# lvxianwei/DeepMerge

Measured on AMD Instinct MI355X. Metric: superpixel-pairs/sec (train step), higher is better.
Workload: dtype bf16; 1 GPU; ShfitScaleFormer_v3 depth [3, 2, 1], scales [32, 64, 128, 256] x 4ch (256x256x4 patches), 32 pairs/GPU/step, fwd+loss+bwd+allreduce+Adam (BASELINE configs[1]); pairs_per_gpu=32, global_batch=32, parallelism=dp1

## Files before the change

### deepmerge_amd/csrc/dm_gemm.hip

```cpp
#include <cstdlib>

#include "dm_common.h"
#include <cstring>

#include "dm_gemm_common.h"
#include "dm_mfma.h"
#include "dm_prof.h"

bool dm_gemm256_plan(GemmParams &p, int layout, int ab_dtype, bool can_split, long long workspace_bytes, int user_split);
void dm_gemm256_launch(const GemmParams &p, int layout, hipStream_t s);
int dm_gemm_ring_plan(GemmParams &p, int layout, int ab_dtype, bool aligned8);
void dm_gemm_ring_launch(const GemmParams &p, int wm, hipStream_t s);
int dm_gemm_w4_plan(GemmParams &p, int layout, int ab_dtype, bool aligned8, bool can_split, long long workspace_bytes);
void dm_gemm_w4_launch(const GemmParams &p, int layout, int grid, hipStream_t s);
int dm_gemm_w4_grouped(GemmParams *ps, int n, hipStream_t s, bool launch, const DmGroupedExtra &x);
long long dm_gemm_w4_grouped_ws_bytes();

namespace {

constexpr int BM = 128, BN = 128;
constexpr int STAGE_BYTES = 16896;
constexpr int NTHREADS = 256;
#ifndef DM_GEMM_LDS_STAGES
#define DM_GEMM_LDS_STAGES 1
#endif
constexpr int LDS_STAGES = DM_GEMM_LDS_STAGES;
constexpr int WG_PER_CU = (LDS_STAGES == 1) ? 3 : 2;


template <typename T, int TM> struct Geo {
  static constexpr int EPC = DmTypeInfo<T>::kPerChunk;
  static constexpr int TILE = 32 * TM;
  static constexpr int BK = 128 / (int)sizeof(T);
  static constexpr int M_ROWB = (sizeof(T) == 2) ? TILE * 2 : (TILE + 4) * 4;
  static constexpr int M_CPR = TILE / EPC;
  static constexpr int M_RPI = NTHREADS / M_CPR;
  static constexpr int K_BYTES = TILE * 128;
  static constexpr int STAGE = (K_BYTES > BK * M_ROWB) ? K_BYTES : BK * M_ROWB;
};

template <int TM> __device__ __forceinline__ int tr_swz(int k) {
  if constexpr (TM == 4) return (k & 3) | (((k >> 3) & 1) << 2);
  else return ((k >> 1) & 1) | (((k >> 3) & 1) << 1);
}

template <int TM> struct OperandView {
  __amdgpu_buffer_rsrc_t rsrc;
  const void *base;
  long long tail_bytes;
  unsigned voff[TM];
  unsigned chunk_k;
};

__device__ __forceinline__ int clamp_records(long long bytes) {
  return (int)(bytes < 0 ? 0 : (bytes > 0x7fffffffLL ? 0x7fffffffLL : bytes));
}

template <typename T, int TM>
__device__ __forceinline__ OperandView<TM> view_kmajor(const T *base, long long ld, int row0, int rows, int K, int t) {
  constexpr int EPC = DmTypeInfo<T>::kPerChunk;
  OperandView<TM> v;
  const int nrows = min(32 * TM, rows - row0);
  const long long bytes = ((long long)(nrows - 1) * ld + K) * (long long)sizeof(T);
  v.rsrc = __builtin_amdgcn_make_buffer_rsrc(const_cast<T *>(base + (long long)row0 * ld), 0, clamp_records(bytes), 0x00020000);
  v.base = nullptr;
  v.tail_bytes = 0;
  v.chunk_k = (t & 7) * EPC;
#pragma unroll
  for (int i = 0; i < TM; ++i) {
    const int row = (t >> 3) + 32 * i;
    const long long off = ((long long)row * ld + v.chunk_k) * (long long)sizeof(T);
    v.voff[i] = (row < nrows) ? (unsigned)off : 0x80000000u;
  }
  return v;
}
template <typename T, int TM>
__device__ __forceinline__ void load_kmajor(u32x4 (&r)[TM], const OperandView<TM> &v, int k0, int kend, long long kphys) {
  const unsigned kill = ((int)(k0 + v.chunk_k) < kend) ? 0u : 0x80000000u;
  const unsigned soff = (unsigned)kphys * (unsigned)sizeof(T);
#pragma unroll
  for (int i = 0; i < TM; ++i) r[i] = __builtin_amdgcn_raw_buffer_load_b128(v.rsrc, v.voff[i] | kill, soff, 0);
}
template <int TM> __device__ __forceinline__ void store_kmajor(char *lds, const u32x4 (&r)[TM], int t) {
  const int c = t & 7;
#pragma unroll
  for (int i = 0; i < TM; ++i) {
    const int row = (t >> 3) + 32 * i;
    *reinterpret_cast<u32x4 *>(lds + row * 128 + ((c ^ (row & 7)) << 4)) = r[i];
  }
}
template <typename T, int TM>
__device__ __forceinline__ OperandView<TM> view_mmajor(const T *base, long long ld, int col0, int cols, int K, int t) {
  using G = Geo<T, TM>;
  OperandView<TM> v;
  v.base = base + col0;
  v.tail_bytes = ((long long)(K - 1) * ld + (cols - col0)) * (long long)sizeof(T);
  v.rsrc = __builtin_amdgcn_make_buffer_rsrc(const_cast<T *>(base), 0, 0, 0x00020000);
  v.chunk_k = 0;
  const int col = (t % G::M_CPR) * G::EPC;
#pragma unroll
  for (int i = 0; i < TM; ++i) {
    const long long k = t / G::M_CPR + G::M_RPI * i;
    v.voff[i] = (col0 + col < cols) ? (unsigned)((k * ld + col) * (long long)sizeof(T)) : 0x80000000u;
  }
  return v;
}
template <typename T, int TM>
__device__ __forceinline__ void load_mmajor(u32x4 (&r)[TM], const OperandView<TM> &v, long long ld, int k0, long long seg_off = 0) {
  const long long skip = (long long)k0 * ld * (long long)sizeof(T);
  const __amdgpu_buffer_rsrc_t rs = __builtin_amdgcn_make_buffer_rsrc(
      const_cast<char *>(reinterpret_cast<const char *>(v.base) + skip + seg_off * (long long)sizeof(T)), 0, clamp_records(v.tail_bytes - skip), 0x00020000);
#pragma unroll
  for (int i = 0; i < TM; ++i) r[i] = __builtin_amdgcn_raw_buffer_load_b128(rs, v.voff[i], 0, 0);
}
template <typename T, int TM> __device__ __forceinline__ void store_mmajor(char *lds, const u32x4 (&r)[TM], int t) {
  using G = Geo<T, TM>;
  const int c = t % G::M_CPR;
#pragma unroll
  for (int i = 0; i < TM; ++i) {
    const int k = t / G::M_CPR + G::M_RPI * i;
    if constexpr (sizeof(T) == 2)
      *reinterpret_cast<u32x4 *>(lds + k * G::M_ROWB + (((c >> 1) ^ tr_swz<TM>(k)) << 5) + ((c & 1) << 4)) = r[i];
    else
      *reinterpret_cast<u32x4 *>(lds + k * G::M_ROWB + (c << 4)) = r[i];
  }
}

__device__ __forceinline__ u32x4 frag_kmajor(const char *lds, int row, int kb, int lane) {
  const int chunk = kb * 4 + (lane >> 4);
  return *reinterpret_cast<const u32x4 *>(lds + row * 128 + ((chunk ^ (row & 7)) << 4));
}
template <typename T, int TM> __device__ __forceinline__ u32x4 frag_mmajor(const char *lds, int col0, int kb, int lane) {
  using G = Geo<T, TM>;
  const int g = lane >> 4;
  u32x4 out;
  if constexpr (sizeof(T) == 2) {
    const int q = (lane >> 2) & 3, p = lane & 3;
    const int col = col0 + 4 * p;
#pragma unroll
    for (int half = 0; half < 2; ++half) {
      const int k = kb * 32 + 8 * g + 4 * half + q;
      const u32x2 w = dm_ds_read_tr16(lds + k * G::M_ROWB + (((col >> 4) ^ tr_swz<TM>(k)) << 5) + ((col & 15) << 1));
      out[2 * half] = w[0];
      out[2 * half + 1] = w[1];
    }
  } else {
    const int i = lane & 15;
#pragma unroll
    for (int j = 0; j < 4; ++j) {
      const int k = kb * 16 + 4 * g + j;
      out[j] = *reinterpret_cast<const unsigned int *>(lds + k * G::M_ROWB + ((col0 + i) << 2));
    }
  }
  return out;
}

template <typename T, int LAYOUT, int TM, bool FOLD = false>
__global__ __launch_bounds__(NTHREADS, (TM == 4 ? WG_PER_CU : 4)) void gemm_kernel(const GemmParams p) {
  using G = Geo<T, TM>;
  constexpr bool A_MMAJOR = (LAYOUT == DM_TN);
  constexpr bool B_MMAJOR = (LAYOUT != DM_NT);
  constexpr int BK = G::BK;
  constexpr int TILE = G::TILE, WT = 16 * TM;
  __shared__ __attribute__((aligned(16))) char smem[2 * LDS_STAGES * G::STAGE];
  auto ldsA = [&](int buf) -> char * { return smem + (2 * (buf % LDS_STAGES)) * G::STAGE; };
// ... 270 lines not shown
    }
    dm_gemm_emit8(p, lo, hi, dm_gemm_row(p, m), n);
  }
}

__global__ void colsum_rows_reduce_kernel(const float *__restrict__ rows, float *__restrict__ out, int M, int R, int accumulate) {
  const int m = blockIdx.x * blockDim.x + threadIdx.x;
  if (m >= M) return;
  float s0 = accumulate ? out[m] : 0.f, s1 = 0.f, s2 = 0.f, s3 = 0.f;
  int r = 0;
  for (; r + 3 < R; r += 4) {
    s0 += rows[(long long)r * M + m];
    s1 += rows[(long long)(r + 1) * M + m];
    s2 += rows[(long long)(r + 2) * M + m];
    s3 += rows[(long long)(r + 3) * M + m];
  }
  for (; r < R; ++r) s0 += rows[(long long)r * M + m];
  out[m] = (s0 + s1) + (s2 + s3);
}

__device__ __forceinline__ void sgemm_small_emit(const GemmParams &p, int m, int n, float v) {
  if (p.bias) v += p.bias[n];
  const long long ro = (long long)m;
  if (p.epilogue == DM_EPI_GELU) {
    if (p.aux) reinterpret_cast<float *>(p.aux)[ro * p.ldaux + n] = v;
    v = dm_gelu(v);
  } else if (p.epilogue == DM_EPI_DGELU) {
    v *= dm_dgelu(reinterpret_cast<const float *>(p.aux)[ro * p.ldaux + n]);
  } else if (p.epilogue == DM_EPI_GELU_GRAD) {
    reinterpret_cast<float *>(p.aux)[ro * p.ldaux + n] = dm_dgelu(v);
    v = dm_gelu(v);
  } else if (p.epilogue == DM_EPI_MUL) {
    v *= reinterpret_cast<const float *>(p.aux)[ro * p.ldaux + n];
  }
  if (p.residual) v += p.residual[ro * p.ldr + n];
  float *c = reinterpret_cast<float *>(p.C) + ro * p.ldc + n;
  if (p.accumulate) v += *c;
  *c = v;
}

template <int LAYOUT, int NW = 4>
__global__ __launch_bounds__(64 * NW) void sgemm_small_kernel(const GemmParams p) {
  __shared__ float sa[NW][32][17], sb[NW][32][17];
  __shared__ float red[NW][16][17];
  const int lane = threadIdx.x & 63, w = threadIdx.x >> 6;
  const int m0 = blockIdx.y * 16, n0 = blockIdx.x * 16;
  const float *A = reinterpret_cast<const float *>(p.A);
  const float *B = reinterpret_cast<const float *>(p.B);
  const int kz0 = gridDim.z > 1 ? blockIdx.z * p.k_per_split : 0, kz1 = gridDim.z > 1 ? min(p.K, kz0 + p.k_per_split) : p.K;
  const int kq = ((kz1 - kz0 + NW - 1) / NW + 31) / 32 * 32;
  const int kbeg = kz0 + w * kq, kend = min(kz1, kbeg + kq);
  const int tx = lane & 15, ty = lane >> 4;
  float acc[4] = {0.f, 0.f, 0.f, 0.f};
  float ra[8], rb[8];
  auto gload = [&](int k0) {
#pragma unroll
    for (int i = 0; i < 8; ++i) {
      const int idx = lane + 64 * i;
      {
        const int r = (LAYOUT == DM_TN) ? (idx & 15) : (idx >> 5), kk = (LAYOUT == DM_TN) ? (idx >> 4) : (idx & 31);
        const int m = m0 + r, k = k0 + kk;
        float v = 0.f;
        if (m < p.M && k < kend) v = (LAYOUT == DM_TN) ? A[(long long)k * p.lda + m] : A[(long long)m * p.lda + k];
        ra[i] = v;
      }
      {
        const int c = (LAYOUT == DM_NT) ? (idx >> 5) : (idx & 15), kk = (LAYOUT == DM_NT) ? (idx & 31) : (idx >> 4);
        const int n = n0 + c, k = k0 + kk;
        float v = 0.f;
        if (n < p.N && k < kend) v = (LAYOUT == DM_NT) ? B[(long long)n * p.ldb + k] : B[(long long)k * p.ldb + n];
        rb[i] = v;
      }
    }
  };
  auto lstore = [&]() {
#pragma unroll
    for (int i = 0; i < 8; ++i) {
      const int idx = lane + 64 * i;
      const int ar = (LAYOUT == DM_TN) ? (idx & 15) : (idx >> 5), ak = (LAYOUT == DM_TN) ? (idx >> 4) : (idx & 31);
      sa[w][ak][ar] = ra[i];
      const int bc = (LAYOUT == DM_NT) ? (idx >> 5) : (idx & 15), bk = (LAYOUT == DM_NT) ? (idx & 31) : (idx >> 4);
      sb[w][bk][bc] = rb[i];
    }
  };
  const int nk = (kq + 31) / 32;
  gload(kbeg);
  for (int it = 0; it < nk; ++it) {
    __syncthreads();
    lstore();
    __syncthreads();
    if (it + 1 < nk) gload(kbeg + (it + 1) * 32);
#pragma unroll
    for (int kk = 0; kk < 32; ++kk) {
      const float bv = sb[w][kk][tx];
#pragma unroll
      for (int j = 0; j < 4; ++j) acc[j] = fmaf(sa[w][kk][4 * ty + j], bv, acc[j]);
    }
  }
#pragma unroll
  for (int j = 0; j < 4; ++j) red[w][4 * ty + j][tx] = acc[j];
  __syncthreads();
  if (threadIdx.x >= 256) return;
  const int om = threadIdx.x >> 4, on = threadIdx.x & 15;
  const int m = m0 + om, n = n0 + on;
  if (m >= p.M || n >= p.N) return;
  float v = (red[0][om][on] + red[1][om][on]) + (red[2][om][on] + red[3][om][on]);
  if constexpr (NW > 4) {
#pragma unroll
    for (int q = 4; q < NW; q += 4) v += (red[q][om][on] + red[q + 1][om][on]) + (red[q + 2][om][on] + red[q + 3][om][on]);
  }
  if (gridDim.z > 1) {
    p.workspace[((long long)blockIdx.z * p.M + m) * p.N + n] = v;
    return;
  }
  sgemm_small_emit(p, m, n, v);
}

__global__ __launch_bounds__(256) void sgemm_small_reduce_kernel(const GemmParams p, int slices) {
  const long long i = (long long)blockIdx.x * 256 + threadIdx.x, mn = (long long)p.M * p.N;
  if (i >= mn) return;
  float v = p.workspace[i];
  int z = 1;
  for (; z + 8 <= slices; z += 8) {
    float t[8];
#pragma unroll
    for (int u = 0; u < 8; ++u) t[u] = p.workspace[(z + u) * mn + i];
#pragma unroll
    for (int u = 0; u < 8; ++u) v += t[u];
  }
  for (; z < slices; ++z) v += p.workspace[z * mn + i];
  sgemm_small_emit(p, (int)(i / p.N), (int)(i % p.N), v);
}

template <typename T, int TM>
void launch_mfma(const GemmParams &p, int layout, int grid, hipStream_t s) {
  if constexpr (sizeof(T) == 2) {
    if (p.k_fold > 0) {
      switch (layout) {
        case DM_NT: hipLaunchKernelGGL((gemm_kernel<T, DM_NT, TM, true>), dim3(grid), dim3(NTHREADS), 0, s, p); break;
        case DM_NN: hipLaunchKernelGGL((gemm_kernel<T, DM_NN, TM, true>), dim3(grid), dim3(NTHREADS), 0, s, p); break;
        default: hipLaunchKernelGGL((gemm_kernel<T, DM_TN, TM, true>), dim3(grid), dim3(NTHREADS), 0, s, p); break;
      }
      return;
    }
  }
  switch (layout) {
    case DM_NT: hipLaunchKernelGGL((gemm_kernel<T, DM_NT, TM>), dim3(grid), dim3(NTHREADS), 0, s, p); break;
    case DM_NN: hipLaunchKernelGGL((gemm_kernel<T, DM_NN, TM>), dim3(grid), dim3(NTHREADS), 0, s, p); break;
    default: hipLaunchKernelGGL((gemm_kernel<T, DM_TN, TM>), dim3(grid), dim3(NTHREADS), 0, s, p); break;
  }
}

struct DmRouteOverride {
  static constexpr int NKEY = 5;
  const char *keys[NKEY] = {"DM_GEMM_W4", "DM_GEMM_W4_TN", "DM_GEMM_RING", "DM_GEMM_256", "DM_GEMM_FORCE_TILE"};
  char saved[NKEY][16];
  bool had[NKEY];
  bool active = false;
  DmRouteOverride(int layout, int M, int N, int K) {
    static const char *const e = getenv("DM_GEMM_ROUTE");
    if (!e || !*e) return;
    char want[64];
    snprintf(want, sizeof(want), "%s:%dx%dx%d=", layout == DM_NT ? "NT" : layout == DM_NN ? "NN" : "TN", M, N, K);
    const char *hit = strstr(e, want);
    if (!hit) return;
    const char *fam = hit + strlen(want);
    const char *vals[NKEY] = {"0", "0", "0", "0", nullptr};
    if (!strncmp(fam, "w4", 2)) { vals[0] = "2"; vals[1] = "2"; }
    else if (!strncmp(fam, "ring", 4)) vals[2] = "2";
    else if (!strncmp(fam, "256", 3)) vals[3] = "2";
    else if (!strncmp(fam, "128", 3)) vals[4] = "128";
    else if (!strncmp(fam, "64", 2)) vals[4] = "64";
    else return;
    active = true;
    for (int i = 0; i < NKEY; ++i) {
      const char *old = getenv(keys[i]);
      had[i] = old != nullptr;
      snprintf(saved[i], sizeof(saved[i]), "%s", old ? old : "");
      if (vals[i]) setenv(keys[i], vals[i], 1); else unsetenv(keys[i]);
    }
  }
  ~DmRouteOverride() {
    if (!active) return;
    for (int i = 0; i < NKEY; ++i) {
      if (had[i]) setenv(keys[i], saved[i], 1); else unsetenv(keys[i]);
    }
  }
};

inline int pick_tile(int layout, int M, int N, int K) {
  if (const char *f = getenv("DM_GEMM_FORCE_TILE")) {
    const int v = atoi(f);
    if (v == 64 || v == 128) return v;
  }
  const long long t128 = (long long)((M + 127) / 128) * ((N + 127) / 128);
  if (t128 >= 256) return 128;
  return (layout == DM_TN && K > 4096 && t128 >= 64) ? 128 : 64;
}

int choose_split(int tiles, int K, int bk) {
  int s = 1;
  while (tiles * s < 256 * WG_PER_CU && s < 32 && K / (s * 2) >= 8 * bk) s *= 2;
  return s;
}

inline int plan_fwd_split(int layout, int M, int N, int K, int &tile) {
  tile = 0;
  static const int mode = [] { const char *e = getenv("DM_GEMM_FWD_SPLIT"); return e ? atoi(e) : 1; }();
  if (mode == 0 || layout == DM_TN || N % 8 != 0 || K < 1536) return 1;
  const long long t128 = (long long)((M + 127) / 128) * ((N + 127) / 128);
  if (t128 >= 256) return 1;
  int split = 4;
  while (split > 1 && K / split < 8 * 64) split >>= 1;
  if (split <= 1) return 1;
  if (t128 * split >= 512) return 1;
  tile = 64;
  return split;
}

}

static int64_t colsum_region_floats(int M) {
  const int64_t fused = 128LL * M, alone = dm_colsum_partial_floats(M);
  return (fused > alone ? fused : alone) + 64;
}

extern "C" int64_t dm_gemm_workspace_bytes(int32_t layout, int32_t M, int32_t N, int32_t K) {
  if (layout != DM_TN) {
    const long long t128 = (long long)((M + 127) / 128) * ((N + 127) / 128);
    const long long t16 = (long long)((M + 15) / 16) * ((N + 15) / 16);
    const int64_t skinny = (K >= 1024 && t16 <= 128) ? (int64_t)32 * M * N * 4 : 0;
    const int64_t sliced = (N % 8 == 0 && K >= 1536 && t128 < 256) ? (int64_t)4 * M * N * 4 : 0;
    return skinny > sliced ? skinny : sliced;
  }
  const int tile = pick_tile(layout, M, N, K);
  const int tiles = ((M + tile - 1) / tile) * ((N + tile - 1) / tile);
  const int s = choose_split(tiles, K, 32);
  return (s > 1 ? (int64_t)s * M * N * 4 : 0) + colsum_region_floats(M) * 4;
}

extern "C" int dm_gemm(const DmGemmArgs *a, void *stream) {
  DM_REQUIRE(a != nullptr, DM_ERR_BAD_SHAPE, "dm_gemm: null args");
  DM_REQUIRE(a->M > 0 && a->N > 0 && a->K > 0, DM_ERR_BAD_SHAPE, "dm_gemm: M,N,K must be positive (got %d,%d,%d)", a->M, a->N, a->K);
  DM_REQUIRE(a->layout >= DM_NT && a->layout <= DM_TN, DM_ERR_BAD_SHAPE, "dm_gemm: bad layout %d", a->layout);
  DM_REQUIRE(a->ab_dtype == DM_F32 || a->ab_dtype == DM_BF16, DM_ERR_BAD_DTYPE, "dm_gemm: bad ab_dtype %d", a->ab_dtype);
  DM_REQUIRE(a->c_dtype == DM_F32 || a->c_dtype == DM_BF16 || a->c_dtype == DM_BF16_PAIR, DM_ERR_BAD_DTYPE, "dm_gemm: bad c_dtype %d", a->c_dtype);
  if (a->c_dtype == DM_BF16_PAIR)
    DM_REQUIRE(a->layout != DM_TN && !a->accumulate && a->split_k <= 1 && a->c_plane > 0 && a->c_plane % 8 == 0 && a->ldc % 8 == 0 && a->N % 8 == 0 &&
                   a->ab_dtype == DM_BF16 && a->rows_per_group == 0,
               DM_ERR_UNSUPPORTED, "dm_gemm: a plane-pair result needs an NT / NN bf16 product without accumulate, N, ldc and c_plane multiples of 8");
  DM_REQUIRE(a->A && a->B && a->C, DM_ERR_BAD_SHAPE, "dm_gemm: null operand");
  DM_REQUIRE(!(a->accumulate && a->c_dtype != DM_F32), DM_ERR_BAD_DTYPE, "dm_gemm: accumulate needs an fp32 C");
  DM_REQUIRE(!(a->accumulate && (a->epilogue == DM_EPI_DGELU || a->epilogue == DM_EPI_MUL)), DM_ERR_UNSUPPORTED,
             "dm_gemm: accumulate cannot be combined with an aux-reading epilogue (DM_EPI_DGELU / DM_EPI_MUL)");
  DM_REQUIRE(a->epilogue == DM_EPI_NONE || a->epilogue == DM_EPI_GELU || a->aux != nullptr, DM_ERR_BAD_SHAPE,
             "dm_gemm: this epilogue needs aux (only DM_EPI_GELU may run without one: inference)");
  hipStream_t s = reinterpret_cast<hipStream_t>(stream);

  GemmParams p{};
  p.A = a->A; p.B = a->B; p.C = a->C; p.bias = a->bias; p.residual = a->residual; p.aux = a->aux;
  p.lda = a->lda; p.ldb = a->ldb; p.ldc = a->ldc; p.ldr = a->ldr; p.ldaux = a->ldaux;
  p.group_stride = a->group_stride; p.rows_per_group = a->rows_per_group;
  p.M = a->M; p.N = a->N; p.K = a->K;
  p.epilogue = a->epilogue; p.accumulate = a->accumulate; p.c_dtype = a->c_dtype; p.aux_dtype = a->aux_dtype;

  p.c_plane = a->c_dtype == DM_BF16_PAIR ? a->c_plane : 0;
  p.k_fold = 0;
  if (a->k_fold > 0) {
    DM_REQUIRE(a->ab_dtype == DM_BF16 && a->K == 3 * a->k_fold && a->k_fold % 64 == 0, DM_ERR_UNSUPPORTED,
               "dm_gemm: k_fold needs bf16 operands, K == 3 * k_fold and k_fold %% 64 == 0 (K=%d k_fold=%d)", a->K, a->k_fold);
    for (int sgm = 0; sgm < 3; ++sgm) {
      DM_REQUIRE(a->a_fold[sgm] >= 0 && a->a_fold[sgm] < (1LL << 30) && a->b_fold[sgm] >= 0 && a->b_fold[sgm] < (1LL << 30) &&
                     a->a_fold[sgm] % 8 == 0 && a->b_fold[sgm] % 8 == 0,
                 DM_ERR_UNSUPPORTED, "dm_gemm: k_fold segment offsets must be multiples of 8 in [0, 2^30)");
      p.a_fold[sgm] = a->a_fold[sgm];
      p.b_fold[sgm] = a->b_fold[sgm];
    }
    p.k_fold = a->k_fold;
  }
  const bool folded = p.k_fold > 0;
  float *cs_region = nullptr;
  int64_t slab_bytes = a->workspace_bytes;
  if (a->colsum_a) {
    DM_REQUIRE(a->layout == DM_TN, DM_ERR_UNSUPPORTED, "dm_gemm: colsum_a goes with DM_TN (column sums of A = dy)");
    const int64_t need = colsum_region_floats(a->M) * 4;
    DM_REQUIRE(a->workspace != nullptr && a->workspace_bytes >= need, DM_ERR_BAD_SHAPE,
               "dm_gemm: colsum_a needs %lld bytes of workspace (got %lld)", (long long)need, (long long)a->workspace_bytes);
    slab_bytes = (a->workspace_bytes - need) & ~15LL;
    cs_region = reinterpret_cast<float *>(reinterpret_cast<char *>(a->workspace) + slab_bytes);
  }
  {
    const long long esz = (a->ab_dtype == DM_BF16) ? 2 : 4;
    DM_REQUIRE(128 * a->lda * esz < (1LL << 31) && 128 * a->ldb * esz < (1LL << 31), DM_ERR_BAD_SHAPE,
               "dm_gemm: leading dimensions too large for 32-bit panel offsets (lda=%lld ldb=%lld)", (long long)a->lda, (long long)a->ldb);
  }
  const int epc = (a->ab_dtype == DM_BF16) ? 8 : 4;
  const int a_inner = (a->layout == DM_TN) ? a->M : a->K;
  const int b_inner = (a->layout == DM_NT) ? a->K : a->N;
  const bool mfma_ok = (a_inner % epc == 0) && (b_inner % epc == 0) && (a->lda % epc == 0) && (a->ldb % epc == 0) &&
                       dm_aligned16(a->A) && dm_aligned16(a->B) && (a->N % 4 == 0) && (a->ldc % 4 == 0) &&
                       (a->residual == nullptr || (a->ldr % 4 == 0 && dm_aligned16(a->residual))) &&
                       (a->aux == nullptr || a->ldaux % 4 == 0) && (a->bias == nullptr || dm_aligned16(a->bias)) &&
                       dm_aligned16(a->C) && (a->rows_per_group == 0 || a->group_stride % 4 == 0) &&
                       !(a->ab_dtype == DM_F32 && a->layout != DM_TN && a->rows_per_group == 0 && a->c_dtype == DM_F32 &&
                         (a->aux == nullptr || a->aux_dtype == DM_F32) &&
                         ((a->M + BM - 1) / BM) * ((a->N + BN - 1) / BN) < 16);
  if (!mfma_ok) {
    DM_REQUIRE(!folded && a->c_dtype != DM_BF16_PAIR, DM_ERR_UNSUPPORTED, "dm_gemm: k_fold / a plane-pair result need the MFMA path's alignment (M=%d N=%d K=%d)", a->M, a->N, a->K);
    DM_REQUIRE(a->ab_dtype == DM_F32 && a->c_dtype == DM_F32 && (a->aux == nullptr || a->aux_dtype == DM_F32),
               DM_ERR_BAD_ALIGN, "dm_gemm: shape/alignment needs the generic path, which is fp32-only "
               "(M=%d N=%d K=%d lda=%lld ldb=%lld)", a->M, a->N, a->K, (long long)a->lda, (long long)a->ldb);
    DM_REQUIRE(a->rows_per_group == 0, DM_ERR_UNSUPPORTED, "dm_gemm: grouped rows need the MFMA path");
    dim3 grid((a->N + 15) / 16, (a->M + 15) / 16);
    static const bool skinny_on = [] { const char *e = getenv("DM_GEMM_SKINNY"); return !(e && atoi(e) == 0); }();
    const long long tiles16 = (long long)grid.x * grid.y;
    int slices = 1;
    if (skinny_on && a->workspace && !a->colsum_a && a->K >= 1024 && tiles16 <= 128) {
      slices = (int)(512 / tiles16);
      if (slices > a->K / 128) slices = a->K / 128;
      if (slices > 32) slices = 32;
      while (slices > 1 && (int64_t)slices * a->M * a->N * 4 > slab_bytes) slices >>= 1;
    }
    if (slices > 1) {
      p.workspace = reinterpret_cast<float *>(a->workspace);
      p.k_per_split = ((a->K + slices - 1) / slices + 31) / 32 * 32;
      slices = (a->K + p.k_per_split - 1) / p.k_per_split;
      grid.z = slices;
    }
    switch (a->layout) {
      case DM_NT: hipLaunchKernelGGL((sgemm_small_kernel<DM_NT>), grid, dim3(256), 0, s, p); break;
      case DM_NN: hipLaunchKernelGGL((sgemm_small_kernel<DM_NN>), grid, dim3(256), 0, s, p); break;
      default: hipLaunchKernelGGL((sgemm_small_kernel<DM_TN>), grid, dim3(256), 0, s, p); break;
    }
    if (slices > 1)
      hipLaunchKernelGGL(sgemm_small_reduce_kernel, dim3((unsigned)(((long long)a->M * a->N + 255) / 256)), dim3(256), 0, s, p, slices);
    DM_LAUNCH_CHECK("dm_gemm(generic)");
    if (a->colsum_a) return dm_colsum(a->A, a->ab_dtype, a->lda, a->colsum_a, a->K, a->M, a->colsum_accumulate, cs_region, stream);
    return DM_OK;
  }

  const bool can_split = (a->layout == DM_TN) && a->epilogue == DM_EPI_NONE && !a->bias && !a->residual &&
                         a->c_dtype == DM_F32 && a->rows_per_group == 0 && a->workspace != nullptr && slab_bytes > 0;
  if (a->split_k > 1) {
    DM_REQUIRE(can_split, DM_ERR_UNSUPPORTED, "dm_gemm: split_k needs DM_TN, no epilogue, fp32 C and a workspace");
    DM_REQUIRE((int64_t)a->split_k * a->M * a->N * 4 <= slab_bytes, DM_ERR_BAD_SHAPE,
               "dm_gemm: split_k=%d needs %lld bytes of split-K workspace, got %lld", a->split_k,
               (long long)((int64_t)a->split_k * a->M * a->N * 4), (long long)slab_bytes);
  }
  const bool ring_aligned = (a->ldc % 8 == 0) && (a->aux == nullptr || a->ldaux % 8 == 0) &&
                            (a->rows_per_group == 0 || a->group_stride % 8 == 0) && a->split_k <= 1 && !a->colsum_a;
  p.workspace = reinterpret_cast<float *>(a->workspace);
  const bool w4_ok = (a->layout == DM_TN) ? (a->split_k == 0 && a->ldc % 4 == 0) : ring_aligned;
  const bool fwd_slices_ok = a->layout != DM_TN && a->ab_dtype == DM_BF16 && a->split_k == 0 && ring_aligned && a->N % 8 == 0 &&
                             (a->residual == nullptr || a->ldr % 8 == 0) && a->workspace != nullptr && slab_bytes > 0;
  DmRouteOverride route_guard(a->layout, a->M, a->N, a->K);
  const int w4 = w4_ok ? dm_gemm_w4_plan(p, a->layout, a->ab_dtype, true, a->layout == DM_TN ? can_split : fwd_slices_ok, slab_bytes) : 0;
  const bool persistent = w4 != 0;
  const int ring = persistent ? 0 : dm_gemm_ring_plan(p, a->layout, a->ab_dtype, ring_aligned);
  const bool big = !persistent && !ring && dm_gemm256_plan(p, a->layout, a->ab_dtype, can_split, slab_bytes, a->split_k);
  int tile = w4 ? 1924 : ring ? (ring == 8 ? 2568 : 1288) : big ? 256 : pick_tile(a->layout, a->M, a->N, a->K);
  int split = w4 ? p.split_k : (ring || persistent) ? 1 : p.split_k;
  bool fwd_split = persistent && a->layout != DM_TN && p.split_k > 1;
  if (!big && !ring && !persistent && fwd_slices_ok) {
    int ft;
    const int fs = plan_fwd_split(a->layout, a->M, a->N, a->K, ft);
    if (fs > 1 && (int64_t)fs * a->M * a->N * 4 <= slab_bytes && !getenv("DM_GEMM_FORCE_TILE")) {
      fwd_split = true;
      tile = ft;
    }
  }
  if (!big && !ring && !persistent) {
    p.tiles_m = (a->M + tile - 1) / tile;
    p.tiles_n = (a->N + tile - 1) / tile;
    const int bk = (a->ab_dtype == DM_BF16) ? 64 : 32;
    split = a->split_k;
    if (fwd_split) { int ft; split = plan_fwd_split(a->layout, a->M, a->N, a->K, ft); }
    else if (split == 0) split = can_split ? choose_split(p.tiles_m * p.tiles_n, a->K, bk) : 1;
    if (split > 1)
      while (split > 1 && (int64_t)split * a->M * a->N * 4 > slab_bytes) split >>= 1;
    int kps = ((a->K + split - 1) / split + bk - 1) / bk * bk;
    split = (a->K + kps - 1) / kps;
    p.split_k = split;
    p.k_per_split = kps;
  }
  p.workspace = reinterpret_cast<float *>(a->workspace);
  {
    static const bool rows_off = [] { const char *e = getenv("DM_GEMM_T128_ROWS"); return e && e[0] == '0'; }();
    if (rows_off && !ring) p.debug |= 0x100;
    static const bool touch_off = [] { const char *e = getenv("DM_GEMM_T128_TOUCH"); return e && e[0] == '0'; }();
    if (touch_off) p.debug |= 0x200;
    static const bool lean_off = [] { const char *e = getenv("DM_GEMM_EPI_LEAN"); return e && e[0] == '0'; }();
    if (lean_off) p.debug |= 0x400;
#ifdef DM_GEMM_ABLATE
    { const char *e = getenv("DM_GEMM_NOEPI"); if (e && e[0] == '1') p.debug |= 0x800; }
#endif
  }
  {
    static const int forced = [] { const char *e = getenv("DM_GEMM_GROUP_M"); return e ? atoi(e) : -1; }();
    p.group_m = forced >= 0 ? forced : 8;
  }
  const int grid = p.tiles_m * p.tiles_n * split;
  {
    static const char *kNames[2][3] = {{"gemm_f32_NT", "gemm_f32_NN", "gemm_f32_TN"}, {"gemm_bf16_NT", "gemm_bf16_NN", "gemm_bf16_TN"}};
    const double esz = (a->ab_dtype == DM_BF16) ? 2.0 : 4.0;
    const double csz = (a->c_dtype == DM_BF16) ? 2.0 : 4.0;
    static const bool by_shape = [] { const char *e = getenv("DM_PROF_SHAPES"); return e && e[0] == '1'; }();
    char shaped[64];
    const char *pname = kNames[a->ab_dtype == DM_BF16][a->layout];
    if (by_shape) {
      snprintf(shaped, sizeof(shaped), "%s_%lldx%lldx%lld_e%d%s%s_t%d", pname, (long long)a->M, (long long)a->N, (long long)a->K, a->epilogue,
               a->residual ? "r" : "", a->c_dtype == DM_BF16 ? "h" : "f", tile);
      pname = shaped;
    }
    const double mn = (double)a->M * a->N;
    DmProfScope prof(pname, s, 2.0 * a->M * a->N * a->K,
                     esz * ((double)a->M * a->K + (double)a->N * a->K) + csz * mn * (a->accumulate ? 2.0 : 1.0) +
                         (a->residual ? 4.0 * mn : 0.0) + (a->aux ? ((a->aux_dtype == DM_BF16) ? 2.0 : 4.0) * mn : 0.0));
    const bool cs_t64 = !big && !w4 && !ring && a->layout == DM_TN && a->ab_dtype == DM_BF16 && tile == 64 && a->colsum_a != nullptr && split <= 128;
    p.colsum_slab = ((big || (w4 && a->layout == DM_TN) || cs_t64) && cs_region) ? cs_region : nullptr;
    if (w4) {
      dm_gemm_w4_launch(p, a->layout, w4, s);
    } else if (ring) {
      dm_gemm_ring_launch(p, ring, s);
    } else if (big) {
      dm_gemm256_launch(p, a->layout, s);
    } else if (a->ab_dtype == DM_BF16) {
      if (tile == 128) launch_mfma<bf16_t, 4>(p, a->layout, grid, s); else launch_mfma<bf16_t, 2>(p, a->layout, grid, s);
    } else {
      if (tile == 128) launch_mfma<float, 4>(p, a->layout, grid, s); else launch_mfma<float, 2>(p, a->layout, grid, s);
    }
    if (fwd_split && split > 1) {
      const long long n8 = (long long)a->M * a->N / 8;
      const long long want = (n8 + 255) / 256;
      GemmParams q = p;
      q.split_k = 1;
      hipLaunchKernelGGL(splitk_epilogue_kernel, dim3((unsigned)(want < 4096 ? want : 4096)), dim3(256), 0, s, q, p.workspace, split);
    }
  }
  DM_LAUNCH_CHECK("dm_gemm");
  if (fwd_split) return DM_OK;
  const bool cs_t64 = !big && !w4 && !ring && a->layout == DM_TN && a->ab_dtype == DM_BF16 && tile == 64 && a->colsum_a != nullptr && split <= 128;
  const bool cs_fused = big || (w4 && a->layout == DM_TN) || cs_t64;
  const int cs_rows_per_slice = big ? 4 : 1;
  if (split > 1) {
    const long long n4 = (long long)a->M * a->N / 4;
    const long long want = (n4 + 255) / 256;
    const int rgrid = (int)(want < 2048 ? want : 2048);
    const bool fold_cs = a->colsum_a && cs_fused;
    const int cs_blocks = fold_cs ? (a->M + 255) / 256 : 0;
    hipLaunchKernelGGL(splitk_reduce_kernel, dim3(rgrid + cs_blocks), dim3(256), 0, s, p.workspace,
                       reinterpret_cast<float *>(a->C), (long long)a->ldc, a->M, a->N, split, a->accumulate, rgrid,
                       fold_cs ? cs_region : nullptr, fold_cs ? a->colsum_a : nullptr, a->M, split * cs_rows_per_slice, a->colsum_accumulate);
    DM_LAUNCH_CHECK("dm_gemm(split-k reduce)");
    if (fold_cs) return DM_OK;
  }
  if (a->colsum_a) {
    if (cs_fused) {
      hipLaunchKernelGGL(colsum_rows_reduce_kernel, dim3((a->M + 63) / 64), dim3(64), 0, s, cs_region, a->colsum_a, a->M, split * cs_rows_per_slice,
                         a->colsum_accumulate);
      DM_LAUNCH_CHECK("dm_gemm(colsum reduce)");
    } else if (folded) {
      int accum = a->colsum_accumulate;
      for (int sgm = 0; sgm < 3; ++sgm) {
        bool first = true;
        for (int e = 0; e < sgm; ++e) first = first && a->a_fold[e] != a->a_fold[sgm];
        if (!first) continue;
        const int rc = dm_colsum(reinterpret_cast<const unsigned short *>(a->A) + a->a_fold[sgm], a->ab_dtype, a->lda, a->colsum_a, a->k_fold, a->M, accum, cs_region, stream);
        if (rc != DM_OK) return rc;
        accum = 1;
      }
    } else {
      const int rc = dm_colsum(a->A, a->ab_dtype, a->lda, a->colsum_a, a->K, a->M, a->colsum_accumulate, cs_region, stream);
      if (rc != DM_OK) return rc;
    }
  }
  return DM_OK;
}

extern "C" int64_t dm_gemm_grouped_workspace_bytes(const DmGemmArgs *args, int32_t n) {
  if (args == nullptr || n < 1 || n > 8) return 0;
  const char *menv = getenv("DM_GEMM_GROUPED");
  if (!menv || atoi(menv) != 3) return 0;
  for (int i = 0; i < n; ++i)
    if (args[i].layout != DM_TN || args[i].ab_dtype != DM_BF16 || args[i].M % 256 != 0 || args[i].N % 192 != 0) return 0;
  return dm_gemm_w4_grouped_ws_bytes();
}

extern "C" int dm_gemm_grouped(const DmGemmArgs *args, int32_t n, void *workspace, int64_t workspace_bytes, void *stream) {
  DM_REQUIRE(args != nullptr && n >= 1, DM_ERR_BAD_SHAPE, "dm_gemm_grouped: null args / n < 1");
  hipStream_t s = reinterpret_cast<hipStream_t>(stream);
  bool fast = n <= 8;
  GemmParams ps[8];
  float *cs_rows[8] = {nullptr};
  DmGroupedExtra x{};
  x.ws = (workspace && dm_aligned16(workspace)) ? workspace : nullptr;
  x.ws_bytes = x.ws ? workspace_bytes : 0;
  for (int i = 0; fast && i < n; ++i) {
    const DmGemmArgs &a = args[i];
    fast = a.layout == DM_TN && a.ab_dtype == DM_BF16 && a.c_dtype == DM_F32 && a.epilogue == DM_EPI_NONE && a.split_k == 0 && a.k_fold >= 0 &&
           a.A && a.B && a.C && !a.bias && !a.residual && !a.aux && a.rows_per_group == 0 && a.M > 0 && a.N > 0 && a.K > 0 &&
           a.M % 8 == 0 && a.N % 8 == 0 && a.lda % 8 == 0 && a.ldb % 8 == 0 && a.ldc % 4 == 0 && a.lda >= a.M && a.ldb >= a.N && a.ldc >= a.N &&
           dm_aligned16(a.A) && dm_aligned16(a.B) && dm_aligned16(a.C);
    if (!fast) break;
    GemmParams p{};
    p.A = a.A; p.B = a.B; p.C = a.C;
    p.lda = a.lda; p.ldb = a.ldb; p.ldc = a.ldc; p.ldr = a.ldc; p.ldaux = a.ldc;
    p.M = a.M; p.N = a.N; p.K = a.K;
    p.epilogue = DM_EPI_NONE; p.accumulate = a.accumulate ? 1 : 0; p.c_dtype = DM_F32; p.aux_dtype = DM_F32;
    p.group_m = 8;
    if (a.k_fold > 0) {
      fast = a.K == 3 * a.k_fold && a.k_fold % 64 == 0;
      for (int sgm = 0; fast && sgm < 3; ++sgm) {
        fast = a.a_fold[sgm] >= 0 && a.a_fold[sgm] < (1LL << 30) && a.b_fold[sgm] >= 0 && a.b_fold[sgm] < (1LL << 30) && a.a_fold[sgm] % 8 == 0 && a.b_fold[sgm] % 8 == 0;
        p.a_fold[sgm] = a.a_fold[sgm];
        p.b_fold[sgm] = a.b_fold[sgm];
      }
      if (!fast) break;
      p.k_fold = a.k_fold;
    }
    x.cs_out[i] = a.colsum_a;
    x.cs_acc[i] = a.colsum_accumulate ? 1 : 0;
    {
      int64_t sb = a.workspace ? a.workspace_bytes : 0;
      x.cs_region[i] = nullptr;
      if (a.colsum_a && a.workspace) {
        const int64_t need = colsum_region_floats(a.M) * 4;
        if (a.workspace_bytes >= need) {
          sb = (a.workspace_bytes - need) & ~15LL;
          x.cs_region[i] = reinterpret_cast<float *>(reinterpret_cast<char *>(a.workspace) + sb);
        } else sb = 0;
      }
      x.slab[i] = sb > 0 ? reinterpret_cast<float *>(a.workspace) : nullptr;
      x.slab_bytes[i] = sb;
    }
    if (a.colsum_a) {
      if (!a.colsum_accumulate) {
        p.colsum_slab = a.colsum_a;
      } else {
        const int64_t need = colsum_region_floats(a.M) * 4;
        fast = a.workspace != nullptr && a.workspace_bytes >= need;
        if (!fast) break;
        cs_rows[i] = reinterpret_cast<float *>(reinterpret_cast<char *>(a.workspace) + ((a.workspace_bytes - need) & ~15LL));
        p.colsum_slab = cs_rows[i];
      }
    }
    ps[i] = p;
  }
  const int form = fast ? dm_gemm_w4_grouped(ps, n, s, false, x) : 0;
  if (form != 0) {
    double flops = 0, bytes = 0;
    for (int i = 0; i < n; ++i) {
      flops += 2.0 * args[i].M * args[i].N * args[i].K;
      bytes += 2.0 * ((double)args[i].M * args[i].K + (double)args[i].N * args[i].K) + 4.0 * (double)args[i].M * args[i].N * (args[i].accumulate ? 2.0 : 1.0);
    }
    static const bool by_shape = [] { const char *e = getenv("DM_PROF_SHAPES"); return e && e[0] == '1'; }();
    char shaped[64];
    const char *pname = "gemm_bf16_TN";
    if (by_shape) {
      snprintf(shaped, sizeof(shaped), "gemm_bf16_TN_grouped%d_K%d_%s", n, args[0].K, form == 2 ? "streamk" : form == 3 ? "sliced" : "1slice");
      pname = shaped;
    }
    {
      DmProfScope prof(pname, s, flops, bytes);
      dm_gemm_w4_grouped(ps, n, s, true, x);
    }
    if (form == 1)
      for (int i = 0; i < n; ++i)
        if (cs_rows[i])
          hipLaunchKernelGGL(colsum_rows_reduce_kernel, dim3((args[i].M + 63) / 64), dim3(64), 0, s, cs_rows[i], args[i].colsum_a, args[i].M, 1, 1);
    if (form == 3)
      for (int i = 0; i < n; ++i) {
        const DmGemmArgs &a = args[i];
        const int split = ps[i].split_k;
        const long long want = ((long long)a.M * a.N / 4 + 255) / 256;
        const int rgrid = (int)(want < 2048 ? want : 2048);
        const bool fold_cs = a.colsum_a != nullptr;
        const int cs_blocks = fold_cs ? (a.M + 255) / 256 : 0;
        hipLaunchKernelGGL(splitk_reduce_kernel, dim3(rgrid + cs_blocks), dim3(256), 0, s, ps[i].workspace, reinterpret_cast<float *>(a.C), (long long)a.ldc,
                           a.M, a.N, split, a.accumulate, rgrid, fold_cs ? x.cs_region[i] : nullptr, fold_cs ? a.colsum_a : nullptr, a.M, split,
                           a.colsum_accumulate);
      }
    DM_LAUNCH_CHECK("dm_gemm_grouped");
    return DM_OK;
  }
  for (int i = 0; i < n; ++i) {
    const int rc = dm_gemm(&args[i], stream);
    if (rc != DM_OK) return rc;
  }
  return DM_OK;
}
```

Baseline: 6294 pairs/s.

## Add single-stage 128x128 bf16 GEMM path for K=768 at four workgroups per CU

Adds a new GEMM kernel family (q4) for NT/NN bf16 shapes. It uses 128x128 tiles, a single 32 KiB LDS stage loaded via buffer-to-LDS DMA with swizzling, and launch bounds of four workgroups per CU. By default it is routed only for K=768 with many tiles, ahead of the ring and 256 paths. The intent is to gain latency hiding from higher occupancy instead of multi-stage pipelining. In exchange, each K step waits on the load before computing, and a new hand-written asm path takes over those shapes.

New measurement: 6407 pairs/s (median of 6 runs). 1.8% higher.

```diff
diff --git a/deepmerge_amd/csrc/dm_gemm.hip b/deepmerge_amd/csrc/dm_gemm.hip
--- a/deepmerge_amd/csrc/dm_gemm.hip
+++ b/deepmerge_amd/csrc/dm_gemm.hip
@@ -11,6 +11,8 @@
 void dm_gemm256_launch(const GemmParams &p, int layout, hipStream_t s);
 int dm_gemm_ring_plan(GemmParams &p, int layout, int ab_dtype, bool aligned8);
 void dm_gemm_ring_launch(const GemmParams &p, int wm, hipStream_t s);
+bool dm_gemm_q4_plan(GemmParams &p, int layout, int ab_dtype, bool aligned8);
+void dm_gemm_q4_launch(const GemmParams &p, int layout, hipStream_t s);
 int dm_gemm_w4_plan(GemmParams &p, int layout, int ab_dtype, bool aligned8, bool can_split, long long workspace_bytes);
 void dm_gemm_w4_launch(const GemmParams &p, int layout, int grid, hipStream_t s);
 int dm_gemm_w4_grouped(GemmParams *ps, int n, hipStream_t s, bool launch, const DmGroupedExtra &x);
@@ -587,8 +589,8 @@
 }
 
 struct DmRouteOverride {
-  static constexpr int NKEY = 5;
-  const char *keys[NKEY] = {"DM_GEMM_W4", "DM_GEMM_W4_TN", "DM_GEMM_RING", "DM_GEMM_256", "DM_GEMM_FORCE_TILE"};
+  static constexpr int NKEY = 6;
+  const char *keys[NKEY] = {"DM_GEMM_W4", "DM_GEMM_W4_TN", "DM_GEMM_RING", "DM_GEMM_256", "DM_GEMM_FORCE_TILE", "DM_GEMM_Q4"};
   char saved[NKEY][16];
   bool had[NKEY];
   bool active = false;
@@ -600,12 +602,13 @@
     const char *hit = strstr(e, want);
     if (!hit) return;
     const char *fam = hit + strlen(want);
-    const char *vals[NKEY] = {"0", "0", "0", "0", nullptr};
+    const char *vals[NKEY] = {"0", "0", "0", "0", nullptr, "0"};
     if (!strncmp(fam, "w4", 2)) { vals[0] = "2"; vals[1] = "2"; }
     else if (!strncmp(fam, "ring", 4)) vals[2] = "2";
     else if (!strncmp(fam, "256", 3)) vals[3] = "2";
     else if (!strncmp(fam, "128", 3)) vals[4] = "128";
     else if (!strncmp(fam, "64", 2)) vals[4] = "64";
+    else if (!strncmp(fam, "q4", 2)) vals[5] = "2";
     else return;
     active = true;
     for (int i = 0; i < NKEY; ++i) {
@@ -791,12 +794,13 @@
   DmRouteOverride route_guard(a->layout, a->M, a->N, a->K);
   const int w4 = w4_ok ? dm_gemm_w4_plan(p, a->layout, a->ab_dtype, true, a->layout == DM_TN ? can_split : fwd_slices_ok, slab_bytes) : 0;
   const bool persistent = w4 != 0;
-  const int ring = persistent ? 0 : dm_gemm_ring_plan(p, a->layout, a->ab_dtype, ring_aligned);
-  const bool big = !persistent && !ring && dm_gemm256_plan(p, a->layout, a->ab_dtype, can_split, slab_bytes, a->split_k);
-  int tile = w4 ? 1924 : ring ? (ring == 8 ? 2568 : 1288) : big ? 256 : pick_tile(a->layout, a->M, a->N, a->K);
-  int split = w4 ? p.split_k : (ring || persistent) ? 1 : p.split_k;
+  const bool q4 = !persistent && dm_gemm_q4_plan(p, a->layout, a->ab_dtype, ring_aligned && a->split_k <= 1);
+  const int ring = (persistent || q4) ? 0 : dm_gemm_ring_plan(p, a->layout, a->ab_dtype, ring_aligned);
+  const bool big = !persistent && !q4 && !ring && dm_gemm256_plan(p, a->layout, a->ab_dtype, can_split, slab_bytes, a->split_k);
+  int tile = w4 ? 1924 : q4 ? 1284 : ring ? (ring == 8 ? 2568 : 1288) : big ? 256 : pick_tile(a->layout, a->M, a->N, a->K);
+  int split = w4 ? p.split_k : (ring || q4 || persistent) ? 1 : p.split_k;
   bool fwd_split = persistent && a->layout != DM_TN && p.split_k > 1;
-  if (!big && !ring && !persistent && fwd_slices_ok) {
+  if (!big && !ring && !q4 && !persistent && fwd_slices_ok) {
     int ft;
     const int fs = plan_fwd_split(a->layout, a->M, a->N, a->K, ft);
     if (fs > 1 && (int64_t)fs * a->M * a->N * 4 <= slab_bytes && !getenv("DM_GEMM_FORCE_TILE")) {
@@ -804,7 +808,7 @@
       tile = ft;
     }
   }
-  if (!big && !ring && !persistent) {
+  if (!big && !ring && !q4 && !persistent) {
     p.tiles_m = (a->M + tile - 1) / tile;
     p.tiles_n = (a->N + tile - 1) / tile;
     const int bk = (a->ab_dtype == DM_BF16) ? 64 : 32;
@@ -851,10 +855,12 @@
     DmProfScope prof(pname, s, 2.0 * a->M * a->N * a->K,
                      esz * ((double)a->M * a->K + (double)a->N * a->K) + csz * mn * (a->accumulate ? 2.0 : 1.0) +
                          (a->residual ? 4.0 * mn : 0.0) + (a->aux ? ((a->aux_dtype == DM_BF16) ? 2.0 : 4.0) * mn : 0.0));
-    const bool cs_t64 = !big && !w4 && !ring && a->layout == DM_TN && a->ab_dtype == DM_BF16 && tile == 64 && a->colsum_a != nullptr && split <= 128;
+    const bool cs_t64 = !big && !w4 && !ring && !q4 && a->layout == DM_TN && a->ab_dtype == DM_BF16 && tile == 64 && a->colsum_a != nullptr && split <= 128;
     p.colsum_slab = ((big || (w4 && a->layout == DM_TN) || cs_t64) && cs_region) ? cs_region : nullptr;
     if (w4) {
       dm_gemm_w4_launch(p, a->layout, w4, s);
+    } else if (q4) {
+      dm_gemm_q4_launch(p, a->layout, s);
     } else if (ring) {
       dm_gemm_ring_launch(p, ring, s);
     } else if (big) {
@@ -874,7 +880,7 @@
   }
   DM_LAUNCH_CHECK("dm_gemm");
   if (fwd_split) return DM_OK;
-  const bool cs_t64 = !big && !w4 && !ring && a->layout == DM_TN && a->ab_dtype == DM_BF16 && tile == 64 && a->colsum_a != nullptr && split <= 128;
+  const bool cs_t64 = !big && !w4 && !ring && !q4 && a->layout == DM_TN && a->ab_dtype == DM_BF16 && tile == 64 && a->colsum_a != nullptr && split <= 128;
   const bool cs_fused = big || (w4 && a->layout == DM_TN) || cs_t64;
   const int cs_rows_per_slice = big ? 4 : 1;
   if (split > 1) {
diff --git a/deepmerge_amd/csrc/dm_gemm_q4.hip b/deepmerge_amd/csrc/dm_gemm_q4.hip
--- /dev/null
+++ b/deepmerge_amd/csrc/dm_gemm_q4.hip
@@ -0,0 +1,204 @@
+#include <cstdlib>
+
+#include "dm_common.h"
+#include "dm_gemm_common.h"
+#include "dm_mfma.h"
+
+namespace dmq4 {
+
+constexpr int BK = 64, TILE = 128, NTHREADS = 256;
+constexpr int IMG = TILE * 128;
+constexpr int LDS = 2 * IMG;
+static_assert(LDS <= 40 * 1024, "four workgroups per CU: at most 40 KiB of LDS each");
+static_assert(LDS >= 4 * 16 * DM_EPI_PITCH, "epilogue staging (16 rows per wave) must fit the operand images");
+
+__device__ __forceinline__ int tr_swz(int k) { return (k & 3) | (((k >> 3) & 1) << 2); }
+
+__device__ __forceinline__ void zero_pinned(f32x4 &acc, const u32x4 &z) {
+  asm volatile("s_nop 1\n\tv_mfma_f32_16x16x32_bf16 %0, %1, %1, 0" : "=a"(acc) : "v"(z));
+}
+__device__ __forceinline__ void mma_pinned(f32x4 &acc, const u32x4 &a, const u32x4 &b) {
+  asm volatile("s_nop 0\n\tv_mfma_f32_16x16x32_bf16 %0, %1, %2, %0" : "+a"(acc) : "v"(b), "v"(a));
+}
+
+#define DM_Q4_PIECE(base, bytes, skip) \
+  __builtin_amdgcn_make_buffer_rsrc(const_cast<char *>((base) + (skip)), 0, (int)max(0LL, min((bytes) - (skip), 0x7fffffffLL)), 0x00020000)
+#define DM_Q4_DMA(rsrc, dst, voff, soff) \
+  __builtin_amdgcn_raw_ptr_buffer_load_lds(rsrc, (__attribute__((address_space(3))) void *)(dst), 16, voff, soff, 0, 0)
+
+template <int LAYOUT>
+__global__ __launch_bounds__(NTHREADS, 4) void gemm_q4_kernel(const GemmParams p) {
+  constexpr bool B_MMAJOR = (LAYOUT == DM_NN);
+  __shared__ __attribute__((aligned(16))) char smem[LDS];
+  char *const ldsA = smem, *const ldsB = smem + IMG;
+  const int t = threadIdx.x, lane = t & 63;
+  const int wave = __builtin_amdgcn_readfirstlane(t >> 6);
+  const int wm = wave >> 1, wn = wave & 1;
+  const int g = lane >> 4, li = lane & 15;
+
+  int id = dm_xcd_remap(blockIdx.x, gridDim.x);
+  int tm, tn;
+  if (p.group_m > 0) {
+    const int band = id / (p.group_m * p.tiles_n);
+    const int within = id - band * (p.group_m * p.tiles_n);
+    const int gsz = min(p.group_m, p.tiles_m - band * p.group_m);
+    tn = within / gsz;
+    tm = band * p.group_m + (within - tn * gsz);
+  } else {
+    tn = id % p.tiles_n;
+    tm = id / p.tiles_n;
+  }
+  const int m0 = tm * TILE, n0 = tn * TILE;
+  const int nk = p.K / BK;
+
+  const int prow = lane >> 3, csrc = (lane & 7) ^ prow;
+  const char *pa = reinterpret_cast<const char *>(p.A) + (long long)m0 * p.lda * 2;
+  const long long bytesA = ((long long)(min(TILE, p.M - m0) - 1) * p.lda + p.K) * 2;
+  const int voA = (int)((long long)(wave * 8 + prow) * p.lda * 2 + csrc * 16);
+  const char *pb;
+  long long bytesB;
+  int voB;
+  if constexpr (!B_MMAJOR) {
+    pb = reinterpret_cast<const char *>(p.B) + (long long)n0 * p.ldb * 2;
+    bytesB = ((long long)(min(TILE, p.N - n0) - 1) * p.ldb + p.K) * 2;
+    voB = (int)((long long)(wave * 8 + prow) * p.ldb * 2 + csrc * 16);
+  } else {
+    pb = reinterpret_cast<const char *>(p.B) + (long long)n0 * 2;
+    bytesB = ((long long)(p.K - 1) * p.ldb + (p.N - n0)) * 2;
+    const int k = wave * 4 + (lane >> 4);
+    const int col = ((((lane & 15) >> 1) ^ tr_swz(k)) << 4) + ((lane & 1) << 3);
+    voB = (n0 + col < p.N) ? (int)(((long long)k * p.ldb + col) * 2) : (int)0x80000000u;
+  }
+  const long long rowA = 32LL * p.lda * 2, stepB = B_MMAJOR ? 16LL * p.ldb * 2 : 32LL * p.ldb * 2;
+  auto stage = [&](int kt) __attribute__((always_inline)) {
+    long long sa = (long long)kt * (BK * 2);
+    long long sb = B_MMAJOR ? (long long)kt * BK * p.ldb * 2 : (long long)kt * (BK * 2);
+#pragma unroll
+    for (int u = 0; u < 4; ++u) {
+#ifdef __HIP_DEVICE_COMPILE__
+      asm volatile("" : "+s"(sa));
+#endif
+      DM_Q4_DMA(DM_Q4_PIECE(pa, bytesA, sa), ldsA + (wave + 4 * u) * 1024, voA, 0);
+      sa += rowA;
+    }
+#pragma unroll
+    for (int u = 0; u < 4; ++u) {
+#ifdef __HIP_DEVICE_COMPILE__
+      asm volatile("" : "+s"(sb));
+#endif
+      DM_Q4_DMA(DM_Q4_PIECE(pb, bytesB, sb), ldsB + (wave + 4 * u) * 1024, voB, 0);
+      sb += stepB;
+    }
+  };
+
+  auto frag_k = [&](const char *img, int row, int kb) __attribute__((always_inline)) {
+    return *reinterpret_cast<const u32x4 *>(img + row * 128 + (((kb * 4 + g) ^ (row & 7)) << 4));
+  };
+  auto frag_m = [&](const char *img, int col0, int kb) __attribute__((always_inline)) {
+    const int q = (lane >> 2) & 3, pp = lane & 3;
+    u32x4 out;
+#pragma unroll
+    for (int half = 0; half < 2; ++half) {
+      const int k = kb * 32 + 8 * g + 4 * half + q;
+      const u32x2 w = dm_ds_read_tr16(img + k * 256 + (((col0 >> 4) ^ tr_swz(k)) << 5) + (pp << 3));
+      out[2 * half] = w[0];
+      out[2 * half + 1] = w[1];
+    }
+    return out;
+  };
+
+  f32x4 acc[4][4];
+  {
+    u32x4 z;
+    asm volatile("v_mov_b32 %0, 0" : "=v"(z[0]));
+    z[1] = z[2] = z[3] = z[0];
+#pragma unroll
+    for (int i = 0; i < 4; ++i)
+#pragma unroll
+      for (int j = 0; j < 4; ++j) zero_pinned(acc[i][j], z);
+  }
+
+  float tv0 = 0.f, tv1 = 0.f;
+  const int touch_at = (!(p.debug & 0x200) && (p.residual || (p.aux && (p.epilogue == DM_EPI_DGELU || p.epilogue == DM_EPI_MUL)))) ? max(0, nk - 4) : -1;
+
+  stage(0);
+  for (int kt = 0; kt < nk; ++kt) {
+    asm volatile("s_waitcnt vmcnt(0)" ::: "memory");
+    __builtin_amdgcn_s_barrier();
+    __builtin_amdgcn_sched_barrier(0);
+#pragma unroll
+    for (int kb = 0; kb < 2; ++kb) {
+      u32x4 fa[4], fb[4];
+#pragma unroll
+      for (int i = 0; i < 4; ++i) {
+        fa[i] = frag_k(ldsA, wm * 64 + i * 16 + li, kb);
+        if constexpr (B_MMAJOR) fb[i] = frag_m(ldsB, wn * 64 + i * 16, kb);
+        else fb[i] = frag_k(ldsB, wn * 64 + i * 16 + li, kb);
+      }
+      if (kb == 1) {
+        asm volatile("s_waitcnt lgkmcnt(0)" ::: "memory");
+        __builtin_amdgcn_s_barrier();
+        __builtin_amdgcn_sched_barrier(0);
+        if (kt + 1 < nk) stage(kt + 1);
+        if (kt == touch_at) {
+          const int m = m0 + wm * 64 + lane, n = n0 + wn * 64;
+          if (m < p.M && n < p.N) {
+            const DmGemmRow rw = dm_gemm_row(p, m);
+            if (p.residual) {
+              tv0 = p.residual[rw.r + n];
+              if (n + 32 < p.N) tv1 = p.residual[rw.r + n + 32];
+            } else if (p.aux_dtype == DM_F32) {
+              tv0 = reinterpret_cast<const float *>(p.aux)[rw.x + n];
+              if (n + 32 < p.N) tv1 = reinterpret_cast<const float *>(p.aux)[rw.x + n + 32];
+            } else {
+              tv0 = __builtin_bit_cast(float, (unsigned)reinterpret_cast<const unsigned short *>(p.aux)[rw.x + n]);
+            }
+          }
+        }
+        __builtin_amdgcn_sched_barrier(0);
+      }
+#pragma unroll
+      for (int i = 0; i < 4; ++i)
+#pragma unroll
+        for (int j = 0; j < 4; ++j) mma_pinned(acc[i][j], fa[i], fb[j]);
+    }
+  }
+
+  asm volatile("s_nop 7\n\ts_nop 7\n\ts_nop 7" ::: "memory");
+#pragma unroll
+  for (int i = 0; i < 4; ++i)
+#pragma unroll
+    for (int j = 0; j < 4; ++j) asm volatile("" : "+a"(acc[i][j]));
+  asm volatile("" ::"v"(tv0), "v"(tv1));
+  dm_epilogue_rows<4, 16, false, DM_EPI_PITCH, false, true>(p, acc, smem + wave * (16 * DM_EPI_PITCH), m0 + wm * 64, n0 + wn * 64, lane);
+}
+
+}
+
+bool dm_gemm_q4_plan(GemmParams &p, int layout, int ab_dtype, bool aligned8) {
+  const char *env = getenv("DM_GEMM_Q4");
+  const int mode = env ? atoi(env) : 1;
+  if (mode == 0 || (layout != DM_NT && layout != DM_NN) || ab_dtype != DM_BF16 || !aligned8) return false;
+  if (p.K % dmq4::BK != 0 || p.N % 8 != 0 || p.k_fold > 0 || p.c_dtype == DM_BF16_PAIR) return false;
+  if (p.M % 64 != 0) return false;
+  static const bool epi_ab = [] {
+    const char *r = getenv("DM_GEMM_T128_ROWS"), *l = getenv("DM_GEMM_EPI_LEAN");
+    return (r && r[0] == '0') || (l && l[0] == '0');
+  }();
+  if (epi_ab) return false;
+  if (p.residual != nullptr && p.ldr % 8 != 0) return false;
+  if (!dm_epi_key_specialised(dm_epi_lean_key(p, 64))) return false;
+  if (128LL * p.lda * 2 >= (1LL << 31) || 128LL * p.ldb * 2 >= (1LL << 31)) return false;
+  if (mode == 1 && !(p.K == 768 && (long long)((p.M + 127) / 128) * ((p.N + 127) / 128) >= 768 && !(layout == DM_NT && p.N < 2304))) return false;
+  p.tiles_m = (p.M + dmq4::TILE - 1) / dmq4::TILE;
+  p.tiles_n = (p.N + dmq4::TILE - 1) / dmq4::TILE;
+  p.split_k = 1;
+  p.k_per_split = p.K;
+  return true;
+}
+
+void dm_gemm_q4_launch(const GemmParams &p, int layout, hipStream_t s) {
+  const dim3 grid((unsigned)(p.tiles_m * p.tiles_n));
+  if (layout == DM_NN) hipLaunchKernelGGL(dmq4::gemm_q4_kernel<DM_NN>, grid, dim3(dmq4::NTHREADS), 0, s, p);
+  else hipLaunchKernelGGL(dmq4::gemm_q4_kernel<DM_NT>, grid, dim3(dmq4::NTHREADS), 0, s, p);
+}
```
